# adelacvg/diff-vits

Hardware: AMD Instinct MI355X
Metric: mel_frames_per_sec_50step_dpmsolver (higher is better)
Workload: dtype bf16x3 (bf16 MFMA operands split hi+lo, 3 products, fp32 accumulate / fp32 activations); 1 GPU; B=8/GPU, C=80, T=1024, L=256, 50-step DPM-Solver++(2M) multistep, UNet1DConditionModel (128, 256, 384, 512), seeded random-init weights; global_batch=8, concurrent_sub_batches_per_gpu=1, rccl_world_size=1, parallelism=dp1 (batch-sharded, RCCL broadcast of conditioning + all-gather of mels)

## Files before the change

diff-vits_amd/csrc/kernels_conv.hip:

```cpp
#include "dv_common.h"
#include "dv_device.h"
#include "gnx_device.h"

#include <cstdlib>
#include <type_traits>

typedef __attribute__((ext_vector_type(8))) __bf16 bf16x8;
typedef __attribute__((ext_vector_type(16))) float f32x16;

#ifdef DV_GEMM_TRACE
__device__ unsigned long long g_c3_trace[1024 * 16];
__device__ int g_c3_sel = 0;
#define DV_C3TRACE(i) do { if (threadIdx.x == 0 && blockIdx.x < 1024 && (g_c3_sel == 0 || g_c3_sel == CIN)) g_c3_trace[blockIdx.x * 16 + (i)] = __builtin_amdgcn_s_memtime(); } while (0)
extern "C" int dv_debug_c3_trace_select(int cin) {
  hipError_t e = hipMemcpyToSymbol(HIP_SYMBOL(g_c3_sel), &cin, sizeof(cin));
  void* d = nullptr;
  if (e == hipSuccess) e = hipGetSymbolAddress(&d, HIP_SYMBOL(g_c3_trace));
  return (int)(e != hipSuccess ? e : hipMemset(d, 0, sizeof(g_c3_trace)));
}
extern "C" int dv_debug_c3_trace(unsigned long long* host, int n_wg) {
  return (int)hipMemcpyFromSymbol(host, HIP_SYMBOL(g_c3_trace), (size_t)n_wg * 16 * sizeof(unsigned long long));
}
#else
#define DV_C3TRACE(i) do {} while (0)
// ... 496 lines not shown
  const bool padded = p.Tv_out != p.T_out;
  const int tfr = t0 + e_wm * 32;
  const bool m_ok = tfr + l31 < p.Tv_out;
#pragma unroll
  for (int g = 0; g < 4; ++g) {
    const float4 b4 = *reinterpret_cast<const float4*>(s_bias + e_wn * 32 + 4 * lh + 8 * g);
    vv[4 * g] += b4.x; vv[4 * g + 1] += b4.y; vv[4 * g + 2] += b4.z; vv[4 * g + 3] += b4.w;
  }
  if (p.epi == EPI_RESIDUAL) {
    const float* rp = p.res + (size_t)min(m, p.M - 1) * p.ldres + ncol0 + 4 * lh;
#pragma unroll
    for (int g = 0; g < 4; ++g) {
      const float4 a = *reinterpret_cast<const float4*>(rp + 8 * g);
      vv[4 * g] += a.x; vv[4 * g + 1] += a.y; vv[4 * g + 2] += a.z; vv[4 * g + 3] += a.w;
    }
  }
  if (padded) {
#pragma unroll
    for (int r = 0; r < 16; ++r) vv[r] = m_ok ? vv[r] : 0.f;
  }
  if (live) {
    const size_t ob = (size_t)m * p.ldo + ncol0;
    if (p.out) {
#pragma unroll
      for (int g = 0; g < 4; ++g)
        dv_st16(p.out + ob + 4 * lh + 8 * g, make_float4(vv[4 * g], vv[4 * g + 1], vv[4 * g + 2], vv[4 * g + 3]));
    }
    if (p.out_hi) store_planes16(p.out_hi, p.out_lo, ob, lh, vv);
  }
  DV_C3TRACE(5);
  if (p.stats16 && live) {
    float a1[2] = {0.f, 0.f}, a2[2] = {0.f, 0.f};
#pragma unroll
    for (int r = 0; r < 16; ++r) a1[r >> 3] += vv[r];
    a1[0] = wave_sum64(a1[0]); a1[1] = wave_sum64(a1[1]);
    const float inv = padded ? 1.0f / (float)(16 * min(32, p.Tv_out - tfr)) : (1.0f / 512.0f);
    const float mb[2] = {a1[0] * inv, a1[1] * inv};
#pragma unroll
    for (int r = 0; r < 16; ++r) { const float dv = (!padded || m_ok) ? vv[r] - mb[r >> 3] : 0.f; a2[r >> 3] = fmaf(dv, dv, a2[r >> 3]); }
    a2[0] = wave_sum64(a2[0]); a2[1] = wave_sum64(a2[1]);
    if (lane < 2) {
      const size_t e = (size_t)(mrow0 >> 5) * (p.N >> 4) + (ncol0 >> 4) + lane;
      const float2 val = make_float2(lane ? a1[1] : a1[0], lane ? a2[1] : a2[0]);
      reinterpret_cast<float2*>(p.stats16)[e] = val;
      if (gnx_h)
        __hip_atomic_store(p.gnx.xchg + e, (unsigned long long)__float_as_uint(val.x) | ((unsigned long long)__float_as_uint(val.y) << 32),
                           __ATOMIC_RELAXED, __HIP_MEMORY_SCOPE_SYSTEM);
    }
  }
  DV_C3TRACE(6);
  if (gnx_h) {
    GnxTile t;
    t.M = p.M; t.N = p.N; t.T_out = p.T_out; t.Tv_out = p.Tv_out; t.m0 = m0; t.n0 = n0; t.bm = tl.rows; t.bn = BN;
    t.bq = tl.bq;
    gnx_finish_table<BN>(p.gnx, t, s_gnx, tid, lane, wave, NWV, [&](int) {});
    DV_C3TRACE(7);
    float y[16];
#pragma unroll
    for (int g = 0; g < 4; ++g) {
      const int cl = e_wn * 32 + 4 * lh + 8 * g;
      const float4 sa = *reinterpret_cast<const float4*>(s_gnx.gA + cl);
      const float4 sb = *reinterpret_cast<const float4*>(s_gnx.gB + cl);
      y[4 * g] = fmaf(vv[4 * g], sa.x, sb.x); y[4 * g + 1] = fmaf(vv[4 * g + 1], sa.y, sb.y);
      y[4 * g + 2] = fmaf(vv[4 * g + 2], sa.z, sb.z); y[4 * g + 3] = fmaf(vv[4 * g + 3], sa.w, sb.w);
    }
    if (p.gnx.silu) {
#pragma unroll
      for (int r = 0; r < 16; ++r) y[r] = y[r] * __builtin_amdgcn_rcpf(1.0f + __expf(-y[r]));
    }
    if (padded) {
#pragma unroll
      for (int r = 0; r < 16; ++r) y[r] = m_ok ? y[r] : 0.f;
    }
    if (live) store_planes16(p.gnx.y_hi, p.gnx.y_lo, (size_t)m * p.N + ncol0, lh, y);
  }
  DV_C3TRACE(8);
}

#ifndef DV_C3_EXP
#define DV_C3_EXP 0
#endif
namespace {
constexpr int RS = 8;
constexpr int SLOT_PL = BM * 128, SLOT = 2 * SLOT_PL;
constexpr int S_HALO = RS * SLOT;
constexpr int S_ZERO = S_HALO + 4096;
constexpr int S_TOTAL = S_HALO + SLOT_PL + 4096 + 256;
constexpr int DWS = 6;
constexpr int NT_S = NT + 64;
static_assert(S_TOTAL + 4096 <= 160 * 1024 && RED_BYTES <= RS * SLOT && RS == 8, "ring geometry");
}

__global__ __launch_bounds__(NT_S) void k_conv3s(const GemmParams p) {
  extern __shared__ __attribute__((aligned(1024))) char smem[];
  __shared__ __attribute__((aligned(16))) float s_bias[BN];
  __shared__ GnxShared<BN> s_gnx;
  asm volatile("" ::"s"(p.seg[0].a0_hi), "s"(p.seg[1].a0_hi), "s"(p.seg[1].pad), "s"(p.T_in), "s"(p.w_hi), "s"(p.M), "s"(p.res),
               "s"(p.out_hi), "s"(p.zero_page), "s"(p.ln_u), "s"(p.gnx.xchg), "s"(p.gnx.y_hi), "s"(p.xcd_n), "s"(p.xcd_inv_tn), "s"(p.wf_lo));
  const GemmSeg& sg = p.seg[0];
  const GemmSeg& sh = p.seg[1];
  const int c0 = sg.c0, c1 = sg.c1, CIN = c0 + c1;
  const int d0 = p.nseg > 1 ? sh.c0 : 0, d1 = p.nseg > 1 ? sh.c1 : 0;
  DV_C3TRACE(0);
  C3Tile tl;
  conv3_tile(p, tl, BM);
  const int m0 = tl.m0, n0 = tl.n0, ksel = tl.ksel, t0 = tl.t0;
  const int rmax = min(BM - 1, p.M - 1 - m0);
  const int tid = threadIdx.x, lane = tid & 63, wave = __builtin_amdgcn_readfirstlane(tid >> 6);
  const unsigned a_base = (unsigned)(size_t)smem;
  const int NCH_ALL = CIN >> 6, KPT = CIN >> 4;
  const int NC2_ALL = (d0 + d1) >> 6;
  const bool half = p.sk_mode == 3;
  const int h1 = half ? (((NCH_ALL >> 1) + 1) & ~1) : NCH_ALL, h2 = half ? ((NC2_ALL + 1) >> 1) : NC2_ALL;
  const int CA = ksel ? h1 : 0, NCH = ksel ? NCH_ALL - h1 : h1;
  const int JA = ksel ? h2 : 0, NC2 = ksel ? NC2_ALL - h2 : h2;
  const int NS2 = (NC2 + 1) >> 1;
  const int NCT = NCH + NC2, NSTEP = NCH + NS2;

  if (wave == NWV) {
    glds4(p.bias ? (const void*)(p.bias + n0 + lane) : (const void*)p.zero_page, (unsigned)(size_t)s_bias);
    const int lr = lane >> 3;
    const unsigned sw_e = (unsigned)(((lane & 7) ^ swz(lr)) << 4), sw_o = (unsigned)(((lane & 7) ^ swz(8 + lr)) << 4);
    auto issue_chunk = [&](int cc) {
      const bool seg0 = cc < NCH;
      const int cb = (seg0 ? CA + cc : JA + cc - NCH) * 64;
      const int e0 = seg0 ? c0 : d0;
      const bool first = cb < e0;
      const int ld = first ? e0 : (seg0 ? c1 : d1);
      const bf16_t* bh = seg0 ? (first ? sg.a0_hi : sg.a1_hi) : (first ? sh.a0_hi : sh.a1_hi);
      const bf16_t* bl = seg0 ? (first ? sg.a0_lo : sg.a1_lo) : (first ? sh.a0_lo : sh.a1_lo);
      const size_t col = (size_t)(first ? cb : cb - e0);
      const unsigned dst = a_base + (unsigned)((cc & (RS - 1)) * SLOT);
#pragma unroll
      for (int r8 = 0; r8 < 8; ++r8) {
        const unsigned vo = (unsigned)((m0 + min(lr + 8 * r8, rmax)) * ld * 2) + ((r8 & 1) ? sw_o : sw_e);
        glds16_s(bh + col, vo, dst + r8 * 1024);
        glds16_s(bl + col, vo, dst + SLOT_PL + r8 * 1024);
      }
    };
    int next = 2;
    for (; next < min(4, NCT); ++next) issue_chunk(next);
    wait_vmcnt<32>();
    __builtin_amdgcn_s_barrier();
    int done = 0;
    for (int s2 = 1; s2 < NSTEP; ++s2) {
      if (!(DV_C3_EXP & 1)) {
        const int lim = min(min(NCT, done + RS), next + 2);
        for (; next < lim; ++next) issue_chunk(next);
      }
      {
        const int s3 = s2 + 1;
        const int need = s3 < NCH ? s3 : min(NCH + 2 * (s3 - NCH) + 1, NCT - 1);
        const int k = next - 1 - need;
        if (k >= 3) wait_vmcnt<48>();
        else if (k == 2) wait_vmcnt<32>();
        else if (k == 1) wait_vmcnt<16>();
        else wait_vmcnt<0>();
      }
      __builtin_amdgcn_s_barrier();
      done += (s2 - 1) < NCH ? 1 : 2;
    }
    return;
  }

  const int l31 = lane & 31, lh = lane >> 5;
  const int cf = wave & 1, kq = wave >> 1;
  const int e_wn = cf, e_wm = (wave >> 1) & 1, e_half = wave >> 2;
  float rpre[8];
  if (p.epi == EPI_RESIDUAL) {
    const float* rp = p.res + (size_t)(m0 + min(e_wm * 32 + l31, rmax)) * p.ldres + n0 + e_wn * 32 + e_half * 16 + 4 * lh;
#pragma unroll
    for (int g = 0; g < 2; ++g) {
      const float4 a = *reinterpret_cast<const float4*>(rp + 8 * g);
      rpre[4 * g] = a.x; rpre[4 * g + 1] = a.y; rpre[4 * g + 2] = a.z; rpre[4 * g + 3] = a.w;
    }
  }
  {
    const int pl = wave & 1, c = (wave >> 1) * 4 + (lane >> 4), which = (lane >> 3) & 1, slot = lane & 7;
    const bool ok = c < NCH_ALL && (which == 0 ? (t0 + BM < p.Tv_out) : (t0 > 0));
    const long srow = which == 0 ? (long)m0 + BM : (long)m0 - 1;
    const int ch = c * 64 + slot * 8;
    const bool first = ch < c0;
    const bf16_t* src = first ? (pl ? sg.a0_lo : sg.a0_hi) : (pl ? sg.a1_lo : sg.a1_hi);
    const void* g = ok ? (const void*)(src + (size_t)srow * (first ? c0 : c1) + (first ? ch : ch - c0)) : (const void*)p.zero_page;
    glds16(g, a_base + (unsigned)(S_HALO + pl * SLOT_PL + (wave >> 1) * 1024));
    if (wave == 0 && lane < 16) *reinterpret_cast<uint4*>(smem + S_ZERO + (lane >> 3) * SLOT_PL + (lane & 7) * 16) = make_uint4(0u, 0u, 0u, 0u);
    const int d_row = wave * 8 + (lane >> 3);
    const unsigned d_sc = (unsigned)(((lane & 7) ^ swz(d_row)) << 4);
#pragma unroll
    for (int cc = 0; cc < 2; ++cc) {
      const int cb = (CA + cc) * 64;
      const bool f0 = cb < c0;
      const unsigned vo = (unsigned)((size_t)(m0 + min(d_row, rmax)) * (f0 ? c0 : c1) * 2) + d_sc;
      const unsigned dst = a_base + (unsigned)(cc * SLOT + wave * 1024);
      glds16_s((f0 ? sg.a0_hi : sg.a1_hi) + (f0 ? cb : cb - c0), vo, dst);
      glds16_s((f0 ? sg.a0_lo : sg.a1_lo) + (f0 ? cb : cb - c0), vo, dst + SLOT_PL);
    }
  }
  const int KSW = 3 * KPT + 4 * NC2_ALL;
  const bf16_t* const wh = p.wf_hi + ((size_t)((n0 >> 5) + cf) * KSW + kq) * 512 + (size_t)lane * 8;
  const bf16_t* const wl = p.wf_lo + ((size_t)((n0 >> 5) + cf) * KSW + kq) * 512 + (size_t)lane * 8;
  auto load_ks = [&](int ks) {
    BFrag f;
    f.h = *reinterpret_cast<const bf16x8*>(wh + (size_t)ks * 512);
    f.l = *reinterpret_cast<const bf16x8*>(wl + (size_t)ks * 512);
    return f;
  };
  auto unit_ks = [&](int c, int t) {
    if (c < NCH) return t * KPT + 4 * (CA + c);
    const int j = 3 * (c - NCH) + t;
    return NC2 > 0 ? 3 * KPT + 4 * (JA + min(j, NC2 - 1)) : 2 * KPT + 4 * (CA + NCH - 1);
  };
  BFrag bq[DWS];
#pragma unroll
  for (int j = 0; j < DWS; ++j) bq[j] = load_ks(unit_ks(j / 3, j % 3));
  __builtin_amdgcn_sched_barrier(0);
  DV_C3TRACE(1);

  const int zr = p.Tv_out - t0;
  int rb[2][3], sm[2][3];
  bool hs[2][3];
#pragma unroll
  for (int rf = 0; rf < 2; ++rf)
#pragma unroll
    for (int tap = 0; tap < 3; ++tap) {
      const int idx = rf * 32 + l31 + tap - 1, c16 = kq * 2 + lh;
      const bool zero = idx == zr && zr < BM;
      hs[rf][tap] = idx < 0 || idx >= BM;
      rb[rf][tap] = zero ? S_ZERO + (c16 << 4) : hs[rf][tap] ? S_HALO + (idx < 0 ? 128 : 0) + (c16 << 4) : idx * 128 + ((c16 ^ swz(idx)) << 4);
      sm[rf][tap] = zero ? 0 : -1;
    }
  f32x16 acc[2];
#pragma unroll
  for (int rf = 0; rf < 2; ++rf)
#pragma unroll
    for (int r = 0; r < 16; ++r) acc[rf][r] = 0.f;
  auto read_a = [&](int c, int t, bf16x8 (&h)[2], bf16x8 (&l)[2]) __attribute__((always_inline)) {
    const int s_slot = (c & (RS - 1)) * SLOT, s_halo = (CA + c) * 256;
#pragma unroll
    for (int rf = 0; rf < 2; ++rf) {
      const bool any_halo = (rf == 0 && t == 0) || (rf == 1 && t == 2);
      const int off = rb[rf][t] + (((any_halo && hs[rf][t]) ? s_halo : s_slot) & sm[rf][t]);
      h[rf] = *reinterpret_cast<const bf16x8*>(smem + off);
      l[rf] = *reinterpret_cast<const bf16x8*>(smem + off + SLOT_PL);
    }
  };
  auto mma = [&](const BFrag& f, bf16x8 (&ah)[2], bf16x8 (&al)[2]) __attribute__((always_inline)) {
    acc[0] = __builtin_amdgcn_mfma_f32_32x32x16_bf16(f.h, al[0], acc[0], 0, 0, 0);
    acc[1] = __builtin_amdgcn_mfma_f32_32x32x16_bf16(f.h, al[1], acc[1], 0, 0, 0);
    acc[0] = __builtin_amdgcn_mfma_f32_32x32x16_bf16(f.l, ah[0], acc[0], 0, 0, 0);
    acc[1] = __builtin_amdgcn_mfma_f32_32x32x16_bf16(f.l, ah[1], acc[1], 0, 0, 0);
    acc[0] = __builtin_amdgcn_mfma_f32_32x32x16_bf16(f.h, ah[0], acc[0], 0, 0, 0);
    acc[1] = __builtin_amdgcn_mfma_f32_32x32x16_bf16(f.h, ah[1], acc[1], 0, 0, 0);
  };
  bf16x8 ahb[2][2], alb[2][2];
  wait_vmcnt<2 * DWS>();
  __builtin_amdgcn_s_barrier();
  DV_C3TRACE(2);
  read_a(0, 0, ahb[0], alb[0]);

  auto chunk = [&](const int c, auto par_tag) __attribute__((always_inline)) {
    constexpr int PAR = decltype(par_tag)::value;
    if (c > 0) __builtin_amdgcn_s_barrier();
#pragma unroll
    for (int t = 0; t < 3; ++t) {
      const int cur = (PAR + t) & 1;
      if (t + 1 < 3) read_a(c, t + 1, ahb[cur ^ 1], alb[cur ^ 1]);
      else if (c + 1 < NCH) read_a(c + 1, 0, ahb[cur ^ 1], alb[cur ^ 1]);
      else read_a(c + 1, 1, ahb[cur ^ 1], alb[cur ^ 1]);
      mma(bq[3 * PAR + t], ahb[cur], alb[cur]);
      __builtin_amdgcn_sched_barrier(0);
      if (!(DV_C3_EXP & 2)) bq[3 * PAR + t] = load_ks(unit_ks(c + 2, t));
      __builtin_amdgcn_sched_barrier(0);
    }
  };
  for (int c = 0; c < NCH; c += 2) {
    chunk(c, std::integral_constant<int, 0>{});
    chunk(c + 1, std::integral_constant<int, 1>{});
  }
  auto pair = [&](const int j2, auto pos_tag) __attribute__((always_inline)) {
    constexpr int POS = decltype(pos_tag)::value;
    __builtin_amdgcn_s_barrier();
    const int j = 2 * j2;
    read_a(NCH + j + 1, 1, ahb[1], alb[1]);
    mma(bq[2 * POS], ahb[0], alb[0]);
    __builtin_amdgcn_sched_barrier(0);
    if (!(DV_C3_EXP & 2)) bq[2 * POS] = load_ks(3 * KPT + 4 * (JA + min(j + 6, NC2 - 1)));
    __builtin_amdgcn_sched_barrier(0);
    read_a(NCH + j + 2, 1, ahb[0], alb[0]);
    if (j + 1 < NC2) mma(bq[2 * POS + 1], ahb[1], alb[1]);
    __builtin_amdgcn_sched_barrier(0);
    if (!(DV_C3_EXP & 2)) bq[2 * POS + 1] = load_ks(3 * KPT + 4 * (JA + min(j + 7, NC2 - 1)));
    __builtin_amdgcn_sched_barrier(0);
  };
  for (int j2 = 0; j2 < NS2; j2 += 3) {
    pair(j2, std::integral_constant<int, 0>{});
    if (j2 + 1 < NS2) pair(j2 + 1, std::integral_constant<int, 1>{});
    if (j2 + 2 < NS2) pair(j2 + 2, std::integral_constant<int, 2>{});
  }
  DV_C3TRACE(3);
  conv3_finish(p, smem, s_bias, s_gnx, acc, rpre, tl, tid, lane, wave, CIN);
}

static bool g_conv3_on = true;
static int g_conv3_stream = 512;
void conv3_env_refresh() {
  const char* e = getenv("DVITS_CONV3"); g_conv3_on = !(e && e[0] == '0');
  const char* e2 = getenv("DVITS_CONV3_STREAM"); g_conv3_stream = e2 ? atoi(e2) : 512;
}
static const bool g_conv3_env_once = [] { conv3_env_refresh(); return true; }();

bool gemm_conv3_shape_ok(const GemmParams& p) {
  if (!g_conv3_on || p.nseg < 1 || p.nseg > 2 || p.seg[0].taps != 3 || p.seg[0].pad != 1 || p.stride != 1 || p.up_mode != UP_NONE) return false;
  const int cin = p.seg[0].c0 + p.seg[0].c1;
  if (cin < 128 || cin > 1024 || cin % 128 != 0) return false;
  if (p.seg[0].c0 % 64 != 0 || p.seg[0].c1 % 64 != 0 || (p.seg[0].c1 > 0 && !p.seg[0].a1_hi)) return false;
  if (p.nseg == 2) {
    const GemmSeg& s1 = p.seg[1];
    if (s1.taps != 1 || s1.pad != 0 || s1.c0 <= 0 || s1.c0 % 64 != 0 || s1.c1 % 64 != 0 || (s1.c1 > 0 && !s1.a1_hi) || s1.c0 + s1.c1 > 2048) return false;
  }
  const int tv_out = p.Tv_out > 0 ? p.Tv_out : p.T_out, tv_in = p.Tv_in > 0 ? p.Tv_in : p.T_in;
  if (p.T_in != p.T_out || tv_in != tv_out || p.T_virt != tv_out || tv_out > p.T_out || tv_out <= p.T_out - 32) return false;
  if (p.T_out % 32 != 0 || p.N % BN != 0 || p.B <= 0 || p.M != p.B * p.T_out) return false;
  if ((p.epi != EPI_STORE && p.epi != EPI_RESIDUAL) || p.stats || p.rowstat_out || p.ln_stat || p.relu || p.rowmask) return false;
  if ((p.ldo & 7) != 0 || (p.epi == EPI_RESIDUAL && (p.ldres & 3) != 0) || p.force_tile != GT_AUTO) return false;
  return true;
}
int gemm_conv3_row_tiles(const GemmParams& p, int bm) { return p.B * ((p.T_out + bm - 1) / bm); }
int gemm_conv3_split(const GemmParams& p, int n_cu) {
  static const bool on = [] { const char* e = getenv("DVITS_CONV3_SPLIT"); return !(e && e[0] == '0'); }();
  if (!on || n_cu <= 0 || !gemm_conv3_shape_ok(p)) return 0;
  const int cin = p.seg[0].c0 + p.seg[0].c1, nch = cin >> 6, nc2 = p.nseg > 1 ? (p.seg[1].c0 + p.seg[1].c1) >> 6 : 0;
  if (cin <= 512 && cin <= g_conv3_stream && p.nseg == 1) return 0;
  if (2 * gemm_conv3_row_tiles(p, BM) * (p.N / BN) > n_cu || nch < 4 || nch + ((nc2 + 1) >> 1) < 8) return 0;
  return 2;
}
size_t gemm_conv3_split_bytes(const GemmParams& p) { return (size_t)2 * gemm_conv3_row_tiles(p, BM) * (p.N / BN) * BM * BN * sizeof(float); }
bool gemm_conv3_up_ok(const GemmParams& p) {
  if (!g_conv3_on || p.nseg != 1 || p.seg[0].taps != 3 || p.seg[0].pad != 1 || p.stride != 1 || p.up_mode != UP_X2) return false;
  const int cin = p.seg[0].c0 + p.seg[0].c1;
  if (cin != 128 && cin != 256 && cin != 384 && cin != 512) return false;
  if (p.seg[0].c0 % 64 != 0 || p.seg[0].c1 % 64 != 0 || (p.seg[0].c1 > 0 && !p.seg[0].a1_hi)) return false;
  const int tv_out = p.Tv_out > 0 ? p.Tv_out : p.T_out, tv_in = p.Tv_in > 0 ? p.Tv_in : p.T_in;
  if (tv_out != 2 * tv_in || p.T_virt != tv_out || tv_out > p.T_out || tv_out <= p.T_out - 32 || tv_in > p.T_in) return false;
  if (p.T_out % 32 != 0 || p.N % BN != 0 || p.B <= 0 || p.M != p.B * p.T_out) return false;
  if ((p.epi != EPI_STORE && p.epi != EPI_RESIDUAL) || p.stats || p.rowstat_out || p.ln_stat || p.relu || p.rowmask) return false;
  if ((p.ldo & 7) != 0 || (p.epi == EPI_RESIDUAL && (p.ldres & 3) != 0) || p.force_tile != GT_AUTO || p.sk_buf) return false;
  return true;
}
int gemm_conv3_k(const GemmParams& p) {
  return 3 * (p.seg[0].c0 + p.seg[0].c1) + (p.nseg > 1 ? p.seg[1].c0 + p.seg[1].c1 : 0);
}
static void conv3_geometry(GemmParams& p, int bm) {
  p.c3_tu = (p.T_out + bm - 1) / bm;
  p.c3_tu_magic = p.c3_tu <= 1 ? 0u : (unsigned)(((1ull << 32) + (unsigned)p.c3_tu - 1) / (unsigned)p.c3_tu);
}

template <int CIN>
static hipError_t conv3_launch(const GemmParams& p, hipStream_t st) {
  constexpr int smem = ConvGeom<CIN>::SMEM;
  hipLaunchKernelGGL((k_conv3<CIN>), dim3(gemm_conv3_row_tiles(p, BM) * (p.N / BN)), dim3(NT), smem, st, p);
  return hipGetLastError();
}
template <int CIN>
static hipError_t conv3_attr() {
  return hipFuncSetAttribute(reinterpret_cast<const void*>(k_conv3<CIN>), hipFuncAttributeMaxDynamicSharedMemorySize, ConvGeom<CIN>::SMEM);
}
template <int CIN>
static hipError_t conv3u_attr() {
  return hipFuncSetAttribute(reinterpret_cast<const void*>(k_conv3u<CIN>), hipFuncAttributeMaxDynamicSharedMemorySize, ConvGeomU<CIN>::SMEM);
}
template <int CIN>
static hipError_t conv3u_launch(const GemmParams& p, hipStream_t st) {
  constexpr int smem = ConvGeomU<CIN>::SMEM;
  hipLaunchKernelGGL((k_conv3u<CIN>), dim3(gemm_conv3_row_tiles(p, BMU) * (p.N / BN)), dim3(NT), smem, st, p);
  return hipGetLastError();
}
hipError_t launch_conv3_up(const GemmParams& pin, hipStream_t st) {
  GemmParams p = pin;
  if (!p.wf_hi || !p.wf_lo || !gemm_conv3_up_ok(p) || p.Kp != 3 * (p.seg[0].c0 + p.seg[0].c1) || p.sk_mode != 0) return hipErrorInvalidValue;
  if (p.Tv_out <= 0) p.Tv_out = p.T_out;
  if (p.Tv_in <= 0) p.Tv_in = p.T_in;
  conv3_geometry(p, BMU);
  if (p.xcd_n > 0) p.xcd_n = 0;
  switch (p.seg[0].c0 + p.seg[0].c1) {
    case 128: return conv3u_launch<128>(p, st);
    case 256: return conv3u_launch<256>(p, st);
    case 384: return conv3u_launch<384>(p, st);
    default: return conv3u_launch<512>(p, st);
  }
}
hipError_t conv3_init() {
  hipError_t e;
  if ((e = conv3u_attr<128>()) != hipSuccess) return e;
  if ((e = conv3u_attr<256>()) != hipSuccess) return e;
  if ((e = conv3u_attr<384>()) != hipSuccess) return e;
  if ((e = conv3u_attr<512>()) != hipSuccess) return e;
  if ((e = hipFuncSetAttribute(reinterpret_cast<const void*>(k_conv3s), hipFuncAttributeMaxDynamicSharedMemorySize, S_TOTAL)) != hipSuccess) return e;
  if ((e = conv3_attr<128>()) != hipSuccess) return e;
  if ((e = conv3_attr<256>()) != hipSuccess) return e;
  if ((e = conv3_attr<384>()) != hipSuccess) return e;
  return conv3_attr<512>();
}
hipError_t launch_conv3(const GemmParams& pin, hipStream_t st) {
  GemmParams p = pin;
  if (!p.wf_hi || !p.wf_lo || !gemm_conv3_shape_ok(p) || p.Kp != gemm_conv3_k(p) || (p.sk_mode != 0 && p.sk_mode != 3)) return hipErrorInvalidValue;
  if (p.Tv_out <= 0) p.Tv_out = p.T_out;
  if (p.Tv_in <= 0) p.Tv_in = p.T_in;
  conv3_geometry(p, BM);
  const int tiles = gemm_conv3_row_tiles(p, BM) * (p.N / BN);
  if (p.sk_mode == 3) {
    if (!p.sk_buf || !p.sk_ticket || p.sk_split != 2 || p.seg[0].c0 + p.seg[0].c1 < 256) return hipErrorInvalidValue;
    hipLaunchKernelGGL(k_conv3s, dim3(2 * tiles), dim3(NT_S), S_TOTAL, st, p);
    return hipGetLastError();
  }
  const int cin = p.seg[0].c0 + p.seg[0].c1;
  if (cin > 512 || cin > g_conv3_stream || p.nseg > 1) {
    hipLaunchKernelGGL(k_conv3s, dim3(tiles), dim3(NT_S), S_TOTAL, st, p);
    return hipGetLastError();
  }
  switch (cin) {
    case 128: return conv3_launch<128>(p, st);
    case 256: return conv3_launch<256>(p, st);
    case 384: return conv3_launch<384>(p, st);
    default: return conv3_launch<512>(p, st);
  }
}
```

Baseline: 67010 mel-frames/s.

## Add hybrid conv3 kernel with resident 3-tap A tile and streamed 1x1 segment

Adds a k_conv3h variant for small per-workgroup channel counts (2, 4 or 8 64-channel chunks). It preloads the whole 3-tap input tile plus halo rows into LDS. The fused 1x1 skip segment, when present, is streamed through a ring buffer filled by a dedicated producer wave. Dispatch sends eligible split-K and two-segment conv3 launches to this kernel instead of the generic streaming kernel. The aim is to drop per-chunk staging and synchronisation for the 3-tap part. The cost is more LDS per workgroup, which may lower occupancy, and added code complexity.

```diff
diff --git a/diff-vits_amd/csrc/kernels_conv.hip b/diff-vits_amd/csrc/kernels_conv.hip
--- a/diff-vits_amd/csrc/kernels_conv.hip
+++ b/diff-vits_amd/csrc/kernels_conv.hip
@@ -822,9 +822,278 @@
   conv3_finish(p, smem, s_bias, s_gnx, acc, rpre, tl, tid, lane, wave, CIN);
 }
 
+namespace {
+template <int RCH>
+struct HybGeom {
+  static constexpr int H_PL = RCH * CHP;
+  static constexpr int RS2 = RCH == 2 ? 7 : RCH == 4 ? 5 : 0;
+  static constexpr int S_RING = 2 * H_PL;
+  static constexpr int S_ZERO = S_RING + RS2 * SLOT;
+  static constexpr int TOTAL = RS2 > 0 ? S_ZERO + SLOT_PL + 256 : S_RING;
+  static_assert((RCH == 2 || RCH == 4 || RCH == 8) && S_RING % 1024 == 0 && TOTAL + 4096 <= 160 * 1024 && RED_BYTES <= TOTAL, "hybrid geometry");
+};
+}
+
+template <int RCH>
+__global__ __launch_bounds__(NT_S) void k_conv3h(const GemmParams p) {
+  using H = HybGeom<RCH>;
+  constexpr int RS2 = H::RS2;
+  extern __shared__ __attribute__((aligned(1024))) char smem[];
+  __shared__ __attribute__((aligned(16))) float s_bias[BN];
+  __shared__ GnxShared<BN> s_gnx;
+  asm volatile("" ::"s"(p.seg[0].a0_hi), "s"(p.seg[1].a0_hi), "s"(p.seg[1].pad), "s"(p.T_in), "s"(p.w_hi), "s"(p.M), "s"(p.res),
+               "s"(p.out_hi), "s"(p.zero_page), "s"(p.ln_u), "s"(p.gnx.xchg), "s"(p.gnx.y_hi), "s"(p.xcd_n), "s"(p.xcd_inv_tn), "s"(p.wf_lo));
+  const GemmSeg& sg = p.seg[0];
+  const GemmSeg& sh = p.seg[1];
+  const int c0 = sg.c0, c1 = sg.c1, CIN = c0 + c1;
+  const int d0 = (RS2 > 0 && p.nseg > 1) ? sh.c0 : 0, d1 = (RS2 > 0 && p.nseg > 1) ? sh.c1 : 0;
+  DV_C3TRACE(0);
+  C3Tile tl;
+  conv3_tile(p, tl, BM);
+  const int m0 = tl.m0, n0 = tl.n0, ksel = tl.ksel, t0 = tl.t0;
+  const int rmax = min(BM - 1, p.M - 1 - m0);
+  const int tid = threadIdx.x, lane = tid & 63, wave = __builtin_amdgcn_readfirstlane(tid >> 6);
+  const unsigned a_base = (unsigned)(size_t)smem;
+  const int NCH_ALL = CIN >> 6, KPT = CIN >> 4;
+  const int NC2_ALL = (d0 + d1) >> 6;
+  const bool half = p.sk_mode == 3;
+  const int h1 = half ? (((NCH_ALL >> 1) + 1) & ~1) : NCH_ALL, h2 = half ? ((NC2_ALL + 1) >> 1) : NC2_ALL;
+  const int CA = ksel ? h1 : 0, NCH = ksel ? NCH_ALL - h1 : h1;
+  const int JA = ksel ? h2 : 0, NC2 = ksel ? NC2_ALL - h2 : h2;
+  const int NS2 = (NC2 + 1) >> 1;
+
+  if (wave == NWV) {
+    glds4(p.bias ? (const void*)(p.bias + n0 + lane) : (const void*)p.zero_page, (unsigned)(size_t)s_bias);
+    if constexpr (RS2 == 0) {
+      wait_vmcnt<0>();
+      __builtin_amdgcn_s_barrier();
+      return;
+    } else {
+      const int lr = lane >> 3;
+      const unsigned sw_e = (unsigned)(((lane & 7) ^ swz(lr)) << 4), sw_o = (unsigned)(((lane & 7) ^ swz(8 + lr)) << 4);
+      auto issue_chunk = [&](int j) {
+        const int cb = (JA + j) * 64;
+        const bool first = cb < d0;
+        const int ld = first ? d0 : d1;
+        const bf16_t* bh = first ? sh.a0_hi : sh.a1_hi;
+        const bf16_t* bl = first ? sh.a0_lo : sh.a1_lo;
+        const size_t col = (size_t)(first ? cb : cb - d0);
+        const unsigned dst = a_base + (unsigned)(H::S_RING + (j % RS2) * SLOT);
+#pragma unroll
+        for (int r8 = 0; r8 < 8; ++r8) {
+          const unsigned vo = (unsigned)((m0 + min(lr + 8 * r8, rmax)) * ld * 2) + ((r8 & 1) ? sw_o : sw_e);
+          glds16_s(bh + col, vo, dst + r8 * 1024);
+          glds16_s(bl + col, vo, dst + SLOT_PL + r8 * 1024);
+        }
+      };
+      int next = 0;
+      const int fill = min(NC2, RS2);
+      for (; next < min(fill, 3); ++next) issue_chunk(next);
+      wait_vmcnt<48>();
+      __builtin_amdgcn_s_barrier();
+      if (NC2 == 0) return;
+      for (; next < fill; ++next) { wait_vmcnt<32>(); issue_chunk(next); }
+      auto landed = [&](int need) {
+        const int k = next - 1 - need;
+        if (k >= 3) wait_vmcnt<48>();
+        else if (k == 2) wait_vmcnt<32>();
+        else if (k == 1) wait_vmcnt<16>();
+        else wait_vmcnt<0>();
+      };
+      landed(0);
+      __builtin_amdgcn_s_barrier();
+      int done = 0;
+      for (int i = 1; i <= NS2; ++i) {
+        const int lim = min(NC2, done + RS2);
+        for (; next < lim; ++next) { wait_vmcnt<32>(); issue_chunk(next); }
+        landed(min(2 * i, NC2 - 1));
+        __builtin_amdgcn_s_barrier();
+        if (i >= 2) done += 2;
+      }
+      return;
+    }
+  }
+
+  const int l31 = lane & 31, lh = lane >> 5;
+  const int cf = wave & 1, kq = wave >> 1;
+  const int e_wn = cf, e_wm = (wave >> 1) & 1, e_half = wave >> 2;
+  float rpre[8];
+  if (p.epi == EPI_RESIDUAL) {
+    const float* rp = p.res + (size_t)(m0 + min(e_wm * 32 + l31, rmax)) * p.ldres + n0 + e_wn * 32 + e_half * 16 + 4 * lh;
+#pragma unroll
+    for (int g = 0; g < 2; ++g) {
+      const float4 a = *reinterpret_cast<const float4*>(rp + 8 * g);
+      rpre[4 * g] = a.x; rpre[4 * g + 1] = a.y; rpre[4 * g + 2] = a.z; rpre[4 * g + 3] = a.w;
+    }
+  }
+  uint4 hv = make_uint4(0u, 0u, 0u, 0u);
+  int h_dst = -1;
+  if (tid < 32 * RCH) {
+    const int pl = tid / (16 * RCH), rem = tid - pl * (16 * RCH), which = rem / (8 * RCH), piece = rem - which * (8 * RCH);
+    const int c = piece >> 3, slot = piece & 7;
+    if (c < NCH) {
+      const int ch = (CA + c) * 64 + slot * 8;
+      const bool ok = which == 0 ? (t0 + BM < p.Tv_out) : (t0 > 0);
+      const long srow = which == 0 ? (long)m0 + BM : (long)m0 - 1;
+      const bool first = ch < c0;
+      const bf16_t* src = first ? (pl ? sg.a0_lo : sg.a0_hi) : (pl ? sg.a1_lo : sg.a1_hi);
+      if (ok) hv = *reinterpret_cast<const uint4*>(src + (size_t)srow * (first ? c0 : c1) + (first ? ch : ch - c0));
+      h_dst = pl * H::H_PL + c * CHP + (BM + which) * 128 + ((slot ^ swz(BM + which)) << 4);
+    }
+  }
+  if (RS2 > 0 && wave == 0 && lane < 16) *reinterpret_cast<uint4*>(smem + H::S_ZERO + (lane >> 3) * SLOT_PL + (lane & 7) * 16) = make_uint4(0u, 0u, 0u, 0u);
+  {
+    const int d_row = wave * 8 + (lane >> 3);
+    const unsigned d_sc = (unsigned)(((lane & 7) ^ swz(d_row)) << 4);
+#pragma unroll
+    for (int c = 0; c < RCH; ++c) {
+      if (c < NCH) {
+        const int cb = (CA + c) * 64;
+        const bool f0 = cb < c0;
+        const unsigned vo = (unsigned)((size_t)(m0 + min(d_row, rmax)) * (f0 ? c0 : c1) * 2) + d_sc;
+        const unsigned dst = a_base + (unsigned)(c * CHP + wave * 1024);
+        glds16_s((f0 ? sg.a0_hi : sg.a1_hi) + (f0 ? cb : cb - c0), vo, dst);
+        glds16_s((f0 ? sg.a0_lo : sg.a1_lo) + (f0 ? cb : cb - c0), vo, dst + H::H_PL);
+      }
+    }
+  }
+  const int KSW = 3 * KPT + 4 * NC2_ALL;
+  const bf16_t* const wh = p.wf_hi + ((size_t)((n0 >> 5) + cf) * KSW + kq) * 512 + (size_t)lane * 8;
+  const bf16_t* const wl = p.wf_lo + ((size_t)((n0 >> 5) + cf) * KSW + kq) * 512 + (size_t)lane * 8;
+  auto load_ks = [&](int ks) {
+    BFrag f;
+    f.h = *reinterpret_cast<const bf16x8*>(wh + (size_t)ks * 512);
+    f.l = *reinterpret_cast<const bf16x8*>(wl + (size_t)ks * 512);
+    return f;
+  };
+  auto unit_ks = [&](int c, int t) {
+    if (c < NCH) return t * KPT + 4 * (CA + c);
+    const int j = 3 * (c - NCH) + t;
+    return NC2 > 0 ? 3 * KPT + 4 * (JA + min(j, NC2 - 1)) : 2 * KPT + 4 * (CA + NCH - 1);
+  };
+  BFrag bq[DWS];
+#pragma unroll
+  for (int j = 0; j < DWS; ++j) bq[j] = load_ks(unit_ks(j / 3, j % 3));
+  __builtin_amdgcn_sched_barrier(0);
+  if (h_dst >= 0) *reinterpret_cast<uint4*>(smem + h_dst) = hv;
+  DV_C3TRACE(1);
+
+  const int zr = p.Tv_out - t0;
+  int ro[2][3], rb1[2], sm1[2];
+#pragma unroll
+  for (int rf = 0; rf < 2; ++rf) {
+#pragma unroll
+    for (int tap = 0; tap < 3; ++tap) {
+      const int idx = rf * 32 + l31 + tap - 1, row = idx < 0 ? BM + 1 : idx;
+      ro[rf][tap] = row * 128 + (((kq * 2 + lh) ^ swz(row)) << 4);
+    }
+    const int idx = rf * 32 + l31, c16 = kq * 2 + lh;
+    const bool zero = idx == zr && zr < BM;
+    rb1[rf] = zero ? H::S_ZERO + (c16 << 4) : H::S_RING + idx * 128 + ((c16 ^ swz(idx)) << 4);
+    sm1[rf] = zero ? 0 : -1;
+  }
+  f32x16 acc[2];
+#pragma unroll
+  for (int rf = 0; rf < 2; ++rf)
+#pragma unroll
+    for (int r = 0; r < 16; ++r) acc[rf][r] = 0.f;
+  auto read_r = [&](int c, int t, bf16x8 (&h)[2], bf16x8 (&l)[2]) __attribute__((always_inline)) {
+#pragma unroll
+    for (int rf = 0; rf < 2; ++rf) {
+      const int off = c * CHP + ro[rf][t];
+      h[rf] = *reinterpret_cast<const bf16x8*>(smem + off);
+      l[rf] = *reinterpret_cast<const bf16x8*>(smem + off + H::H_PL);
+    }
+  };
+  auto read_1 = [&](int j, bf16x8 (&h)[2], bf16x8 (&l)[2]) __attribute__((always_inline)) {
+    if constexpr (RS2 > 0) {
+      const int s_slot = (j % RS2) * SLOT;
+#pragma unroll
+      for (int rf = 0; rf < 2; ++rf) {
+        const int off = rb1[rf] + (s_slot & sm1[rf]);
+        h[rf] = *reinterpret_cast<const bf16x8*>(smem + off);
+        l[rf] = *reinterpret_cast<const bf16x8*>(smem + off + SLOT_PL);
+      }
+    } else {
+      read_r(0, 1, h, l);
+    }
+  };
+  auto mma = [&](const BFrag& f, bf16x8 (&ah)[2], bf16x8 (&al)[2]) __attribute__((always_inline)) {
+    acc[0] = __builtin_amdgcn_mfma_f32_32x32x16_bf16(f.h, al[0], acc[0], 0, 0, 0);
+    acc[1] = __builtin_amdgcn_mfma_f32_32x32x16_bf16(f.h, al[1], acc[1], 0, 0, 0);
+    acc[0] = __builtin_amdgcn_mfma_f32_32x32x16_bf16(f.l, ah[0], acc[0], 0, 0, 0);
+    acc[1] = __builtin_amdgcn_mfma_f32_32x32x16_bf16(f.l, ah[1], acc[1], 0, 0, 0);
+    acc[0] = __builtin_amdgcn_mfma_f32_32x32x16_bf16(f.h, ah[0], acc[0], 0, 0, 0);
+    acc[1] = __builtin_amdgcn_mfma_f32_32x32x16_bf16(f.h, ah[1], acc[1], 0, 0, 0);
+  };
+  bf16x8 ahb[2][2], alb[2][2];
+  wait_vmcnt<2 * DWS>();
+  if (zr < BM && (zr >> 3) == wave && (lane >> 3) == (zr & 7)) {
+#pragma unroll
+    for (int c = 0; c < RCH; ++c) {
+      if (c < NCH) {
+        *reinterpret_cast<uint4*>(smem + c * CHP + wave * 1024 + lane * 16) = make_uint4(0u, 0u, 0u, 0u);
+        *reinterpret_cast<uint4*>(smem + H::H_PL + c * CHP + wave * 1024 + lane * 16) = make_uint4(0u, 0u, 0u, 0u);
+      }
+    }
+  }
+  __syncthreads();
+  DV_C3TRACE(2);
+  read_r(0, 0, ahb[0], alb[0]);
+
+  auto chunk = [&](const int c, auto par_tag, auto last_tag) __attribute__((always_inline)) {
+    constexpr int PAR = decltype(par_tag)::value;
+    constexpr bool LAST = decltype(last_tag)::value;
+    if (LAST && RS2 > 0 && NC2 > 0) __builtin_amdgcn_s_barrier();
+#pragma unroll
+    for (int t = 0; t < 3; ++t) {
+      const int cur = (PAR + t) & 1;
+      if (t + 1 < 3) read_r(c, t + 1, ahb[cur ^ 1], alb[cur ^ 1]);
+      else if (!LAST) read_r(c + 1, 0, ahb[cur ^ 1], alb[cur ^ 1]);
+      else read_1(0, ahb[cur ^ 1], alb[cur ^ 1]);
+      mma(bq[3 * PAR + t], ahb[cur], alb[cur]);
+      __builtin_amdgcn_sched_barrier(0);
+      bq[3 * PAR + t] = load_ks(unit_ks(c + 2, t));
+      __builtin_amdgcn_sched_barrier(0);
+    }
+  };
+  for (int c = 0; c < NCH - 2; c += 2) {
+    chunk(c, std::integral_constant<int, 0>{}, std::false_type{});
+    chunk(c + 1, std::integral_constant<int, 1>{}, std::false_type{});
+  }
+  chunk(NCH - 2, std::integral_constant<int, 0>{}, std::false_type{});
+  chunk(NCH - 1, std::integral_constant<int, 1>{}, std::true_type{});
+  if constexpr (RS2 > 0) {
+    auto pair = [&](const int j2, auto pos_tag) __attribute__((always_inline)) {
+      constexpr int POS = decltype(pos_tag)::value;
+      __builtin_amdgcn_s_barrier();
+      const int j = 2 * j2;
+      read_1(j + 1, ahb[1], alb[1]);
+      mma(bq[2 * POS], ahb[0], alb[0]);
+      __builtin_amdgcn_sched_barrier(0);
+      bq[2 * POS] = load_ks(3 * KPT + 4 * (JA + min(j + 6, NC2 - 1)));
+      __builtin_amdgcn_sched_barrier(0);
+      read_1(j + 2, ahb[0], alb[0]);
+      if (j + 1 < NC2) mma(bq[2 * POS + 1], ahb[1], alb[1]);
+      __builtin_amdgcn_sched_barrier(0);
+      bq[2 * POS + 1] = load_ks(3 * KPT + 4 * (JA + min(j + 7, NC2 - 1)));
+      __builtin_amdgcn_sched_barrier(0);
+    };
+    for (int j2 = 0; j2 < NS2; j2 += 3) {
+      pair(j2, std::integral_constant<int, 0>{});
+      if (j2 + 1 < NS2) pair(j2 + 1, std::integral_constant<int, 1>{});
+      if (j2 + 2 < NS2) pair(j2 + 2, std::integral_constant<int, 2>{});
+    }
+  }
+  DV_C3TRACE(3);
+  conv3_finish(p, smem, s_bias, s_gnx, acc, rpre, tl, tid, lane, wave, CIN);
+}
+
 static bool g_conv3_on = true;
 static int g_conv3_stream = 512;
+static int g_conv3_hybrid = 1;
 void conv3_env_refresh() {
+  const char* e3 = getenv("DVITS_CONV3_HYBRID"); g_conv3_hybrid = e3 ? atoi(e3) : 1;
   const char* e = getenv("DVITS_CONV3"); g_conv3_on = !(e && e[0] == '0');
   const char* e2 = getenv("DVITS_CONV3_STREAM"); g_conv3_stream = e2 ? atoi(e2) : 512;
 }
@@ -896,6 +1165,37 @@
   hipLaunchKernelGGL((k_conv3u<CIN>), dim3(gemm_conv3_row_tiles(p, BMU) * (p.N / BN)), dim3(NT), smem, st, p);
   return hipGetLastError();
 }
+template <int RCH>
+static hipError_t conv3h_attr() {
+  return hipFuncSetAttribute(reinterpret_cast<const void*>(k_conv3h<RCH>), hipFuncAttributeMaxDynamicSharedMemorySize, HybGeom<RCH>::TOTAL);
+}
+template <int RCH>
+static hipError_t conv3h_launch(const GemmParams& p, int wgs, hipStream_t st) {
+  hipLaunchKernelGGL((k_conv3h<RCH>), dim3(wgs), dim3(NT_S), HybGeom<RCH>::TOTAL, st, p);
+  return hipGetLastError();
+}
+extern "C" int dv_debug_conv3h_lds(int rch) {
+  return rch == 2 ? HybGeom<2>::TOTAL : rch == 4 ? HybGeom<4>::TOTAL : rch == 8 ? HybGeom<8>::TOTAL : -1;
+}
+static int conv3_hybrid_rch(const GemmParams& p) {
+  const int nch_all = (p.seg[0].c0 + p.seg[0].c1) >> 6;
+  const bool half = p.sk_mode == 3;
+  const int nch = half ? (((nch_all >> 1) + 1) & ~1) : nch_all;
+  if (p.nseg == 1) return (half && nch <= 8 && (g_conv3_hybrid & 1)) ? 8 : 0;
+  if (nch == 2) return (g_conv3_hybrid & 2) ? 2 : 0;
+  if (nch == 4) return (g_conv3_hybrid & (half ? 8 : 4)) ? 4 : 0;
+  return 0;
+}
+static hipError_t conv3_stream_launch(const GemmParams& p, int wgs, hipStream_t st) {
+  switch (conv3_hybrid_rch(p)) {
+    case 2: return conv3h_launch<2>(p, wgs, st);
+    case 4: return conv3h_launch<4>(p, wgs, st);
+    case 8: return conv3h_launch<8>(p, wgs, st);
+    default: break;
+  }
+  hipLaunchKernelGGL(k_conv3s, dim3(wgs), dim3(NT_S), S_TOTAL, st, p);
+  return hipGetLastError();
+}
 hipError_t launch_conv3_up(const GemmParams& pin, hipStream_t st) {
   GemmParams p = pin;
   if (!p.wf_hi || !p.wf_lo || !gemm_conv3_up_ok(p) || p.Kp != 3 * (p.seg[0].c0 + p.seg[0].c1) || p.sk_mode != 0) return hipErrorInvalidValue;
@@ -917,6 +1217,9 @@
   if ((e = conv3u_attr<384>()) != hipSuccess) return e;
   if ((e = conv3u_attr<512>()) != hipSuccess) return e;
   if ((e = hipFuncSetAttribute(reinterpret_cast<const void*>(k_conv3s), hipFuncAttributeMaxDynamicSharedMemorySize, S_TOTAL)) != hipSuccess) return e;
+  if ((e = conv3h_attr<2>()) != hipSuccess) return e;
+  if ((e = conv3h_attr<4>()) != hipSuccess) return e;
+  if ((e = conv3h_attr<8>()) != hipSuccess) return e;
   if ((e = conv3_attr<128>()) != hipSuccess) return e;
   if ((e = conv3_attr<256>()) != hipSuccess) return e;
   if ((e = conv3_attr<384>()) != hipSuccess) return e;
@@ -931,14 +1234,10 @@
   const int tiles = gemm_conv3_row_tiles(p, BM) * (p.N / BN);
   if (p.sk_mode == 3) {
     if (!p.sk_buf || !p.sk_ticket || p.sk_split != 2 || p.seg[0].c0 + p.seg[0].c1 < 256) return hipErrorInvalidValue;
-    hipLaunchKernelGGL(k_conv3s, dim3(2 * tiles), dim3(NT_S), S_TOTAL, st, p);
-    return hipGetLastError();
+    return conv3_stream_launch(p, 2 * tiles, st);
   }
   const int cin = p.seg[0].c0 + p.seg[0].c1;
-  if (cin > 512 || cin > g_conv3_stream || p.nseg > 1) {
-    hipLaunchKernelGGL(k_conv3s, dim3(tiles), dim3(NT_S), S_TOTAL, st, p);
-    return hipGetLastError();
-  }
+  if (cin > 512 || cin > g_conv3_stream || p.nseg > 1) return conv3_stream_launch(p, tiles, st);
   switch (cin) {
     case 128: return conv3_launch<128>(p, st);
     case 256: return conv3_launch<256>(p, st);
```

After: 66970 mel-frames/s, median of 2. About the same (-0.1%).
